# yashsmehta/visreps

Measured on AMD Instinct MI355X. Metric: end-to-end RSA eval sec (extract→RDM→1000-bootstrap Spearman), N=10k stimuli, lower is better.
Workload: dtype bf16x3-split Gram, fp32 accumulate (|dSpearman| < 1e-5 vs fp64 RDMs: tests/test_benchsize.py) / exact int ranks, fp64 statistic

## Files before the change

include/visreps_hip.h:

```cpp
#ifndef VISREPS_HIP_H
#define VISREPS_HIP_H

#include <stddef.h>
#include <stdint.h>

#ifdef __cplusplus
extern "C" {
#endif

#define VR_OK 0
#define VR_EINVAL (-1)
#define VR_EHIP (-2)
#define VR_EWORKSPACE (-3)
#define VR_EINTERNAL (-4)
#define VR_ENOCONV (-5)

int vr_version(void);
const char* vr_last_error(void);

size_t vr_rdm_pearson_workspace(int64_t n, int64_t d);
int vr_rdm_pearson_f32(const float* X, int64_t n, int64_t d, int64_t ldx, float* rdm,
                       int64_t ldr, float correction, void* ws, size_t ws_bytes,
                       void* stream);

// ... 121 lines not shown
                      void* ws, size_t ws_bytes, void* stream);

size_t vr_bootstrap_cka_workspace(int64_t n, int64_t n_sets);
int vr_bootstrap_cka_f32(const float* K, const float* L, int64_t n, int64_t ld,
                         const int32_t* idx, int64_t k, int64_t n_sets, int full_first,
                         double* scores, void* ws, size_t ws_bytes, void* stream);

size_t vr_knn2_workspace(int64_t n, int64_t d);
int vr_knn2_f32(const float* X, int64_t n, int64_t d, int64_t ldx, double* r, int32_t* nn,
                void* ws, size_t ws_bytes, void* stream);
int64_t vr_knn2_last_fallback_rows(void);
int vr_twonn_id_f64(const double* r, int64_t n, double* out, void* stream);

size_t vr_srp_workspace(int64_t B, int64_t D);
int vr_srp_csr_f32(const int32_t* indptr, const int32_t* indices, const float* values,
                   int64_t k, int64_t D, const float* X, int64_t B, int64_t ldx, float* out,
                   int64_t ldo, void* ws, size_t ws_bytes, void* stream);

size_t vr_spearman_full_workspace(int64_t n);
size_t vr_spearman_full_sort_workspace(int64_t n);
int vr_spearman_full_last_form(void);
int vr_spearman_full_f32(const float* A, const float* B, int64_t n, int64_t ld, double* out,
                         void* ws, size_t ws_bytes, void* stream);
int vr_spearman_full_subset_f32(const float* A, const float* B, int64_t n, int64_t ld, const int32_t* idx,
                                int64_t k, double* out, void* ws, size_t ws_bytes, void* stream);
int vr_key_counts_u32(const uint32_t* keys, int64_t m, uint32_t kmin, int64_t bins, uint32_t* cnt, void* stream);
size_t vr_key_table_workspace(int64_t bins);
int vr_key_table_midranks(const uint32_t* keys, int64_t m, uint32_t kmin, uint32_t* cnt, int64_t bins, uint64_t* y,
                          uint64_t* tie, void* ws, size_t ws_bytes, void* stream);
int vr_f32_sort_keys(const float* v, int64_t m, uint32_t* keys, void* stream);
size_t vr_sort_pairs_workspace(int64_t m);
int vr_sort_pairs_u32(uint32_t* keys, uint32_t* vals, int64_t m, void* ws, size_t ws_bytes,
                      void* stream);
size_t vr_midranks_workspace(int64_t m);
int vr_midranks_sorted(const uint32_t* keys, int64_t m, uint64_t base, uint64_t* y, uint64_t* tie,
                       void* ws, size_t ws_bytes, void* stream);
size_t vr_dot_u64_workspace(void);
int vr_dot_u64(const uint64_t* a, const uint64_t* b, int64_t m, uint64_t* out, void* ws,
               size_t ws_bytes, void* stream);

int64_t vr_rdm_plane_rows(int64_t n);
size_t vr_rdm_plane_row_bytes(int64_t d);
int vr_rdm_split_rows_f32(const float* X, int64_t rows, int64_t d, int64_t ldx, float correction,
                          float* mean, float* stdv, uint16_t* planes, void* stream);
int vr_rdm_split_rows_multi_f32(int npts, const float* const* X, const int64_t* d, const int64_t* ldx,
                                int64_t rows, float correction, float* const* mean, float* const* stdv,
                                uint16_t* const* planes, void* stream);
int vr_gather_rows_multi_f32(int npts, const float* const* X, const int64_t* d, const int64_t* ldx,
                             int nrows, const int32_t* src, const int32_t* dst, float* const* out,
                             const int64_t* ldo, void* stream);
size_t vr_rdm_planes_tiles_workspace(int64_t n, int64_t d, int64_t tile_begin, int64_t tile_end);
int vr_rdm_pearson_tiles_planes(const uint16_t* planes, const float* mean, const float* stdv,
                                int64_t n, int64_t d, float* rdm, int64_t ldr, float correction,
                                int64_t tile_begin, int64_t tile_end, void* ws, size_t ws_bytes,
                                void* stream);
int vr_rdm_tiles_pack(const float* rdm, int64_t ldr, int64_t n, int64_t tile_begin,
                      int64_t tile_end, float* packed, void* stream);
int vr_rdm_tiles_unpack(const float* packed, int64_t n, int64_t tile_begin, int64_t tile_end,
                        float* rdm, int64_t ldr, void* stream);

int vr_rccl_available(void);
int vr_rccl_unique_id(void* out );
int vr_rccl_comm_init(void** comm, int world, const void* unique_id, int rank);
int vr_rccl_comm_destroy(void* comm);
int vr_rdm_sharded_range(int64_t n, int64_t d, int world, int rank, int64_t* tile_begin, int64_t* tile_end);
size_t vr_rdm_sharded_workspace(int64_t n, int64_t d, int world);
int vr_rdm_pearson_sharded(const float* X_local, int64_t rows_local, int64_t n, int64_t d, int64_t ldx, float* rdm,
                           int64_t ldr, float correction, void* comm, int rank, int world, void* ws, size_t ws_bytes,
                           void* stream);

typedef int (*vr_allgather_fn)(const void* send, void* recv, size_t bytes, void* user, void* stream);
typedef struct vr_comm {
  int world;
  int rank;
  vr_allgather_fn all_gather;
  void* user;
} vr_comm;
int vr_comm_rccl(vr_comm* out, void* nccl_comm, int world, int rank);
int vr_rdm_pearson_sharded_comm(const float* X_local, int64_t rows_local, int64_t n, int64_t d, int64_t ldx,
                                float* rdm, int64_t ldr, float correction, const vr_comm* comm, void* ws,
                                size_t ws_bytes, void* stream);

size_t vr_transform_workspace(int64_t B, int64_t H, int64_t W, int64_t resize, int64_t crop,
                              int filter);
int vr_transform_u8(const uint8_t* src, int64_t B, int64_t H, int64_t W, int64_t resize,
                    int64_t crop, int filter, const float* mean, const float* std, float* out,
                    void* ws, size_t ws_bytes, void* stream);

int vr_col_sum_f32(const float* X, int64_t n, int64_t p, int64_t ldx, const float* init,
                   float* sum, void* stream);
int vr_col_mean_f32(const float* X, int64_t n, int64_t p, int64_t ldx, float* mean, void* stream);
int vr_mean_from_sum_f32(const float* sum, int64_t p, int64_t n, float* mean, void* stream);
size_t vr_pca_cov_workspace(int64_t n, int64_t p);
int vr_pca_cov_f64(const float* X, int64_t n, int64_t p, int64_t ldx, const float* mean,
                   double denom, double* cov, int64_t ldc, void* ws, size_t ws_bytes,
                   void* stream);

size_t vr_gram64_workspace(int64_t n, int64_t p, int rows);
int vr_gram64_f32(const float* X, int64_t n, int64_t p, int64_t ldx, int rows, double* G, int64_t ldg,
                  void* ws, size_t ws_bytes, void* stream);

int vr_col_mean_f64(const float* X, int64_t n, int64_t p, int64_t ldx, double* mean, void* stream);
size_t vr_centred_gram64_workspace(int64_t n, int64_t p, int rows);
int vr_centred_gram64_f32(const float* X, int64_t n, int64_t p, int64_t ldx, const double* mean,
                          int rows, double denom, double* G, int64_t ldg, void* ws,
                          size_t ws_bytes, void* stream);

size_t vr_eigvalsh_workspace(int64_t m);
int vr_eigvalsh_f64(double* A, int64_t m, int64_t lda, double* w, void* ws, size_t ws_bytes,
                    void* stream);

size_t vr_eigh_top_workspace(int64_t m, int64_t k);
int vr_eigh_top_f64(double* A, int64_t m, int64_t lda, int64_t k, double* w, double* V, int64_t ldv,
                    void* ws, size_t ws_bytes, void* stream);

size_t vr_xgemm_nt_workspace(int64_t M, int64_t N, int64_t K);
int vr_xgemm_nt_f32(const float* A, int64_t M, int64_t K, int64_t lda, const int32_t* a_rows,
                    const double* a_mean, const void* B, int b_f64, int64_t N, int64_t ldb, void* G,
                    int g_f64, int64_t ldg, void* ws, size_t ws_bytes, void* stream);

size_t vr_xcov_segments_workspace(int64_t p, int64_t q, int64_t F, int64_t max_seg);
int vr_xcov_segments_f32(const float* X, int64_t ldx, const float* Y, int64_t ldy, int64_t p, int64_t q,
                         const int32_t* rows, const int64_t* seg, int64_t F, const double* mean_x,
                         const double* mean_y, double* S, double* stats, void* ws, size_t ws_bytes,
                         void* stream);

size_t vr_fold_xcov_workspace(int64_t p, int64_t q);
int vr_fold_xcov_f64(const double* S, const double* stats, const int64_t* seg, int64_t F, int64_t p,
                     int64_t q, const double* mean_x, const double* mean_y, double* C, void* ws,
                     size_t ws_bytes, void* stream);

size_t vr_plssvd_folds_workspace(int64_t p, int64_t q, int64_t k, int64_t max_test);
int vr_plssvd_folds_f64(const float* X, int64_t ldx, const float* Y, int64_t ldy, int64_t p, int64_t q,
                        const int32_t* rows, const int64_t* seg, int64_t F, int64_t n_run,
                        const double* mean_x, const double* mean_y, const double* S, const double* stats,
                        int64_t k, double* corr, double* cov, double* sigma, int32_t* null,
                        double* imbalance, int64_t wfold, double* weights, double* wmean, double* wstd,
                        void* ws, size_t ws_bytes, void* stream);

size_t vr_svd_jacobi_workspace(int64_t batch, int64_t p, int64_t q);
int vr_svd_jacobi_f64(const double* A, int64_t batch, int64_t p, int64_t q, int64_t lda, int64_t stride_a,
                      double* S, double* U, double* Vt, int32_t* null, int32_t* sweeps, void* ws,
                      size_t ws_bytes, void* stream);
int vr_jacobi_schedule(int64_t nb, int32_t* pairs);

size_t vr_plssvd_folds_svd_workspace(int64_t p, int64_t q, int64_t k, int64_t max_test, int64_t n_run);
int vr_plssvd_folds_svd_f64(const float* X, int64_t ldx, const float* Y, int64_t ldy, int64_t p, int64_t q,
                            const int32_t* rows, const int64_t* seg, int64_t F, int64_t n_run,
                            const double* mean_x, const double* mean_y, const double* S, const double* stats,
                            int64_t k, double* corr, double* cov, double* sigma, int32_t* null,
                            double* imbalance, int64_t wfold, double* weights, double* wmean, double* wstd,
                            void* ws, size_t ws_bytes, void* stream);

size_t vr_rng_state_bytes(void);
int vr_rng_seed(void* state, uint32_t seed);
int vr_rng_permutation(void* state, int64_t n, int32_t* out);
int vr_rng_choice(void* state, int64_t n, int64_t k, int32_t* out);
int vr_rng_random_u32(void* state, int64_t count, uint32_t* out);
int vr_rng_normal_f64(void* state, int64_t count, double loc, double scale, double* out);
int vr_legacy_choice(uint32_t seed, int64_t n, int64_t k, int64_t n_draws, int32_t* out);

double vr_percentile_linear(const double* x, int64_t n, double q);

#ifdef __cplusplus
}
#endif

#endif
```

visreps_amd/_lib.py:

```python
from __future__ import annotations

import ctypes
import os
import threading

import torch

__all__ = [
    "LIB_PATH",
    "VisrepsHipError",
    "lib",
    "check",
    "stream_of",
    "workspace",
    "EXPORTED_SYMBOLS",
]

LIB_PATH = os.environ.get("VISREPS_AMD_LIB") or os.path.join(
    os.path.dirname(os.path.abspath(__file__)), "libvisreps_hip.so")


class VisrepsHipError(RuntimeError):
    """A libvisreps_hip call returned a non-zero status."""

# ... 104 lines not shown
        [_vp, _c_i64, _vp, _c_i64, _c_i64, _vp, _c_i64, _c_i64, ctypes.c_int, _vp, _c_i64, _vp, _vp, _c_sz, _vp],
    ),
    "vr_engine_posmap4_bytes": (_c_sz, [_c_i64]),
    "vr_engine_posmap4": (ctypes.c_int, [_vp, _c_i64, _c_i64, _vp, _vp]),
    "vr_engine_join4": (ctypes.c_int, [_vp, _c_i64, _vp, _c_i64, _vp, _vp]),
    "vr_engine_est_reruns": (_c_i64, []),
    "vr_engine_est_tail_flags": (_c_i64, []),
    "vr_test_engine_inject": (ctypes.c_int, [_c_i64]),
    "vr_engine_est_predicted": (_c_i64, []),
    "vr_engine_est1_fallbacks": (_c_i64, []),
    "vr_ktimer_enable": (ctypes.c_int, [ctypes.c_int]),
    "vr_trace_mark": (ctypes.c_int, [ctypes.c_int, ctypes.c_int, _vp]),
    "vr_ktimer_read": (ctypes.c_int, [ctypes.c_int, ctypes.POINTER(ctypes.c_double),
                                      ctypes.POINTER(ctypes.c_int64), ctypes.POINTER(ctypes.c_double)]),
    "vr_bootstrap_spearman_workspace": (_c_sz, [_c_i64]),
    "vr_bootstrap_spearman_f32": (
        ctypes.c_int,
        [_vp, _vp, _c_i64, _c_i64, _vp, _c_i64, _c_i64, ctypes.c_int, _vp, _vp, _c_sz, _vp],
    ),
    "vr_kendall_triu_workspace": (_c_sz, [_c_i64]),
    "vr_kendall_triu_f32": (
        ctypes.c_int,
        [_vp, _vp, _c_i64, _c_i64, _vp, _vp, _c_sz, _vp],
    ),
    "vr_kendall_vec_workspace": (_c_sz, [_c_i64]),
    "vr_kendall_tau_a_f64": (ctypes.c_int, [_vp, _vp, _c_i64, _vp, _vp, _c_sz, _vp]),
    "vr_kendall_full_vec_workspace": (_c_sz, [_c_i64]),
    "vr_kendall_full_vec_f64": (ctypes.c_int, [_vp, _vp, _c_i64, _vp, _vp, _c_sz, _vp]),
    "vr_kendall_full_workspace": (_c_sz, [_c_i64]),
    "vr_kendall_full_f32": (ctypes.c_int, [_vp, _vp, _c_i64, _c_i64, _vp, _vp, _c_sz, _vp]),
    "vr_bootstrap_kendall_workspace": (_c_sz, [_c_i64, _c_i64]),
    "vr_bootstrap_kendall_plans": (
        ctypes.c_int,
        [_vp, _vp, _c_i64, _vp, _c_i64, _c_i64, ctypes.c_int, _vp, _vp, _c_sz, _vp],
    ),
    "vr_srp_workspace": (_c_sz, [_c_i64, _c_i64]),
    "vr_srp_csr_f32": (
        ctypes.c_int,
        [_vp, _vp, _vp, _c_i64, _c_i64, _vp, _c_i64, _c_i64, _vp, _c_i64, _vp, _c_sz, _vp],
    ),
    "vr_col_sum_f32": (ctypes.c_int, [_vp, _c_i64, _c_i64, _c_i64, _vp, _vp, _vp]),
    "vr_col_mean_f32": (ctypes.c_int, [_vp, _c_i64, _c_i64, _c_i64, _vp, _vp]),
    "vr_mean_from_sum_f32": (ctypes.c_int, [_vp, _c_i64, _c_i64, _vp, _vp]),
    "vr_pca_cov_workspace": (_c_sz, [_c_i64, _c_i64]),
    "vr_pca_cov_f64": (
        ctypes.c_int,
        [_vp, _c_i64, _c_i64, _c_i64, _vp, ctypes.c_double, _vp, _c_i64, _vp, _c_sz, _vp],
    ),
    "vr_gram64_workspace": (_c_sz, [_c_i64, _c_i64, ctypes.c_int]),
    "vr_gram64_f32": (ctypes.c_int, [_vp, _c_i64, _c_i64, _c_i64, ctypes.c_int, _vp, _c_i64, _vp, _c_sz, _vp]),
    "vr_col_mean_f64": (ctypes.c_int, [_vp, _c_i64, _c_i64, _c_i64, _vp, _vp]),
    "vr_centred_gram64_workspace": (_c_sz, [_c_i64, _c_i64, ctypes.c_int]),
    "vr_centred_gram64_f32": (
        ctypes.c_int,
        [_vp, _c_i64, _c_i64, _c_i64, _vp, ctypes.c_int, ctypes.c_double, _vp, _c_i64, _vp, _c_sz, _vp],
    ),
    "vr_eigvalsh_workspace": (_c_sz, [_c_i64]),
    "vr_eigvalsh_f64": (ctypes.c_int, [_vp, _c_i64, _c_i64, _vp, _vp, _c_sz, _vp]),
    "vr_eigh_top_workspace": (_c_sz, [_c_i64, _c_i64]),
    "vr_eigh_top_f64": (ctypes.c_int, [_vp, _c_i64, _c_i64, _c_i64, _vp, _vp, _c_i64, _vp, _c_sz, _vp]),
    "vr_spearman_full_workspace": (_c_sz, [_c_i64]),
    "vr_spearman_full_sort_workspace": (_c_sz, [_c_i64]),
    "vr_spearman_full_last_form": (ctypes.c_int, []),
    "vr_key_counts_u32": (ctypes.c_int, [_vp, _c_i64, ctypes.c_uint32, _c_i64, _vp, _vp]),
    "vr_key_table_workspace": (_c_sz, [_c_i64]),
    "vr_key_table_midranks": (ctypes.c_int, [_vp, _c_i64, ctypes.c_uint32, _vp, _c_i64, _vp, _vp, _vp, _c_sz, _vp]),
    "vr_spearman_full_f32": (ctypes.c_int, [_vp, _vp, _c_i64, _c_i64, _vp, _vp, _c_sz, _vp]),
    "vr_spearman_full_subset_f32": (ctypes.c_int, [_vp, _vp, _c_i64, _c_i64, _vp, _c_i64, _vp, _vp, _c_sz, _vp]),
    "vr_kendall_full_subset_f32": (ctypes.c_int, [_vp, _vp, _c_i64, _c_i64, _vp, _c_i64, _vp, _vp, _c_sz, _vp]),
    "vr_f32_sort_keys": (ctypes.c_int, [_vp, _c_i64, _vp, _vp]),
    "vr_sort_pairs_workspace": (_c_sz, [_c_i64]),
    "vr_sort_pairs_u32": (ctypes.c_int, [_vp, _vp, _c_i64, _vp, _c_sz, _vp]),
    "vr_midranks_workspace": (_c_sz, [_c_i64]),
    "vr_midranks_sorted": (ctypes.c_int, [_vp, _c_i64, ctypes.c_uint64, _vp, _vp, _vp, _c_sz, _vp]),
    "vr_dot_u64_workspace": (_c_sz, []),
    "vr_dot_u64": (ctypes.c_int, [_vp, _vp, _c_i64, _vp, _vp, _c_sz, _vp]),
    "vr_rdm_plane_rows": (_c_i64, [_c_i64]),
    "vr_rdm_plane_row_bytes": (_c_sz, [_c_i64]),
    "vr_rdm_split_rows_f32": (
        ctypes.c_int, [_vp, _c_i64, _c_i64, _c_i64, ctypes.c_float, _vp, _vp, _vp, _vp]),
    "vr_rdm_split_rows_multi_f32": (
        ctypes.c_int, [ctypes.c_int, _vp, _vp, _vp, _c_i64, ctypes.c_float, _vp, _vp, _vp, _vp]),
    "vr_gather_rows_multi_f32": (
        ctypes.c_int, [ctypes.c_int, _vp, _vp, _vp, ctypes.c_int, _vp, _vp, _vp, _vp, _vp]),
    "vr_rdm_planes_tiles_workspace": (_c_sz, [_c_i64, _c_i64, _c_i64, _c_i64]),
    "vr_rdm_pearson_tiles_planes": (
        ctypes.c_int,
        [_vp, _vp, _vp, _c_i64, _c_i64, _vp, _c_i64, ctypes.c_float, _c_i64, _c_i64, _vp, _c_sz, _vp],
    ),
    "vr_rccl_available": (ctypes.c_int, []),
    "vr_rccl_unique_id": (ctypes.c_int, [_vp]),
    "vr_rccl_comm_init": (ctypes.c_int, [ctypes.POINTER(ctypes.c_void_p), ctypes.c_int, _vp, ctypes.c_int]),
    "vr_rccl_comm_destroy": (ctypes.c_int, [_vp]),
    "vr_rdm_sharded_range": (ctypes.c_int, [_c_i64, _c_i64, ctypes.c_int, ctypes.c_int,
                                            ctypes.POINTER(ctypes.c_int64), ctypes.POINTER(ctypes.c_int64)]),
    "vr_rdm_sharded_workspace": (_c_sz, [_c_i64, _c_i64, ctypes.c_int]),
    "vr_rdm_pearson_sharded": (
        ctypes.c_int,
        [_vp, _c_i64, _c_i64, _c_i64, _c_i64, _vp, _c_i64, ctypes.c_float, _vp, ctypes.c_int, ctypes.c_int, _vp,
         _c_sz, _vp],
    ),
    "vr_comm_rccl": (ctypes.c_int, [_vp, _vp, ctypes.c_int, ctypes.c_int]),
    "vr_rdm_pearson_sharded_comm": (
        ctypes.c_int,
        [_vp, _c_i64, _c_i64, _c_i64, _c_i64, _vp, _c_i64, ctypes.c_float, _vp, _vp, _c_sz, _vp],
    ),
    "vr_rdm_tiles_pack": (ctypes.c_int, [_vp, _c_i64, _c_i64, _c_i64, _c_i64, _vp, _vp]),
    "vr_rdm_tiles_unpack": (ctypes.c_int, [_vp, _c_i64, _c_i64, _c_i64, _vp, _c_i64, _vp]),
    "vr_transform_workspace": (_c_sz, [_c_i64, _c_i64, _c_i64, _c_i64, _c_i64, ctypes.c_int]),
    "vr_transform_u8": (
        ctypes.c_int,
        [_vp, _c_i64, _c_i64, _c_i64, _c_i64, _c_i64, ctypes.c_int, _vp, _vp, _vp, _vp, _c_sz, _vp],
    ),
    "vr_rng_state_bytes": (_c_sz, []),
    "vr_rng_seed": (ctypes.c_int, [_vp, ctypes.c_uint32]),
    "vr_rng_permutation": (ctypes.c_int, [_vp, _c_i64, _vp]),
    "vr_rng_choice": (ctypes.c_int, [_vp, _c_i64, _c_i64, _vp]),
    "vr_rng_random_u32": (ctypes.c_int, [_vp, _c_i64, _vp]),
    "vr_rng_normal_f64": (ctypes.c_int, [_vp, _c_i64, ctypes.c_double, ctypes.c_double, _vp]),
    "vr_xgemm_nt_workspace": (_c_sz, [_c_i64, _c_i64, _c_i64]),
    "vr_xgemm_nt_f32": (
        ctypes.c_int,
        [_vp, _c_i64, _c_i64, _c_i64, _vp, _vp, _vp, ctypes.c_int, _c_i64, _c_i64, _vp, ctypes.c_int, _c_i64,
         _vp, _c_sz, _vp],
    ),
    "vr_xcov_segments_workspace": (_c_sz, [_c_i64, _c_i64, _c_i64, _c_i64]),
    "vr_xcov_segments_f32": (
        ctypes.c_int,
        [_vp, _c_i64, _vp, _c_i64, _c_i64, _c_i64, _vp, _vp, _c_i64, _vp, _vp, _vp, _vp, _vp, _c_sz, _vp],
    ),
    "vr_fold_xcov_workspace": (_c_sz, [_c_i64, _c_i64]),
    "vr_fold_xcov_f64": (
        ctypes.c_int,
        [_vp, _vp, _vp, _c_i64, _c_i64, _c_i64, _vp, _vp, _vp, _vp, _c_sz, _vp],
    ),
    "vr_plssvd_folds_workspace": (_c_sz, [_c_i64, _c_i64, _c_i64, _c_i64]),
    "vr_plssvd_folds_f64": (
        ctypes.c_int,
        [_vp, _c_i64, _vp, _c_i64, _c_i64, _c_i64, _vp, _vp, _c_i64, _c_i64, _vp, _vp, _vp, _vp, _c_i64,
         _vp, _vp, _vp, _vp, _vp, _c_i64, _vp, _vp, _vp, _vp, _c_sz, _vp],
    ),
    "vr_svd_jacobi_workspace": (_c_sz, [_c_i64, _c_i64, _c_i64]),
    "vr_svd_jacobi_f64": (
        ctypes.c_int,
        [_vp, _c_i64, _c_i64, _c_i64, _c_i64, _c_i64, _vp, _vp, _vp, _vp, _vp, _vp, _c_sz, _vp],
    ),
    "vr_jacobi_schedule": (ctypes.c_int, [_c_i64, _vp]),
    "vr_plssvd_folds_svd_workspace": (_c_sz, [_c_i64, _c_i64, _c_i64, _c_i64, _c_i64]),
    "vr_plssvd_folds_svd_f64": (
        ctypes.c_int,
        [_vp, _c_i64, _vp, _c_i64, _c_i64, _c_i64, _vp, _vp, _c_i64, _c_i64, _vp, _vp, _vp, _vp, _c_i64,
         _vp, _vp, _vp, _vp, _vp, _c_i64, _vp, _vp, _vp, _vp, _c_sz, _vp],
    ),
    "vr_legacy_choice": (ctypes.c_int, [ctypes.c_uint32, _c_i64, _c_i64, _c_i64, _vp]),
    "vr_percentile_linear": (ctypes.c_double, [_vp, _c_i64, ctypes.c_double]),
}

EXPORTED_SYMBOLS = tuple(_PROTOTYPES)

VR_ALLGATHER_FN = ctypes.CFUNCTYPE(ctypes.c_int, _vp, _vp, _c_sz, _vp, _vp)


class VrComm(ctypes.Structure):
    _fields_ = [("world", ctypes.c_int), ("rank", ctypes.c_int), ("all_gather", VR_ALLGATHER_FN), ("user", _vp)]

_lib = None
_lock = threading.Lock()


def lib() -> ctypes.CDLL:
    global _lib
    if _lib is not None:
        return _lib
    with _lock:
        if _lib is None:
            if not os.path.exists(LIB_PATH):
                raise ImportError(
                    f"{LIB_PATH} not found: build the MI355X kernels first "
                    "(python -c 'import __graft_entry__ as g; g.build()' or "
                    "make -C visreps_amd/csrc). There is no CPU fallback."
                )
            handle = ctypes.CDLL(LIB_PATH, mode=ctypes.RTLD_GLOBAL)
            for name, (res, args) in _PROTOTYPES.items():
                fn = getattr(handle, name)
                fn.restype = res
                fn.argtypes = args
            _lib = handle
    return _lib


def check(rc: int, fn: str) -> None:
    if rc != 0:
        msg = lib().vr_last_error().decode(errors="replace")
        raise VisrepsHipError(f"{fn} failed (status {rc}): {msg}")


def stream_of(device: torch.device) -> int:
    return int(torch.cuda.current_stream(device).cuda_stream)


class _WorkspacePool:

    def __init__(self):
        self._bufs: dict[tuple, torch.Tensor] = {}

    def get(self, device: torch.device, nbytes: int, tag: str = "ws") -> torch.Tensor:
        key = (str(device), tag)
        buf = self._bufs.get(key)
        if buf is None or buf.numel() < nbytes:
            self._bufs.pop(key, None)
            buf = torch.empty(max(int(nbytes), 256), dtype=torch.uint8, device=device)
            self._bufs[key] = buf
        return buf

    def current(self, device: torch.device, tag: str = "ws") -> int:
        buf = self._bufs.get((str(device), tag))
        return 0 if buf is None else int(buf.numel())

    def release(self, tag: str | None = None) -> None:
        if tag is None:
            self._bufs.clear()
        else:
            for k in [k for k in self._bufs if k[1] == tag]:
                del self._bufs[k]


workspace = _WorkspacePool()


KTIMER_KERNELS = {"k_rankB_est": 0, "k_rankB_exact": 1, "k_rankA": 2, "k_join": 3,
                  "k_gram_wide": 4, "k_gram_tile": 5, "k_countA": 6, "k_rankB_full": 7,
                  "k_kwalk": 8, "k_cov": 9, "k_join4": 10,
                  "k_full_corr": 11, "k_rankB_grid": 12}
KTIMER_KNN = {"knn_stage": 13, "k_knn_cand": 14, "knn_rerank": 15, "k_knn_exact_rows": 16}

KTIMER_EIG = {"eig_tridiag": 17, "eig_bisect": 18, "eig_invit": 19, "eig_back": 20}

KTIMER_SVD = {"svd_stage": 21, "svd_step": 22, "svd_finish": 23}


def ktimer_enable(on: bool = True) -> None:
    check(lib().vr_ktimer_enable(1 if on else 0), "vr_ktimer_enable")


def ktimer_read(kernel: str) -> tuple[float, int, float]:
    ms, n, u = ctypes.c_double(), ctypes.c_int64(), ctypes.c_double()
    kid = (KTIMER_KERNELS[kernel] if kernel in KTIMER_KERNELS else
           KTIMER_KNN[kernel] if kernel in KTIMER_KNN else
           KTIMER_SVD[kernel] if kernel in KTIMER_SVD else KTIMER_EIG[kernel])
    check(lib().vr_ktimer_read(kid, ctypes.byref(ms), ctypes.byref(n), ctypes.byref(u)),
          "vr_ktimer_read")
    return ms.value, n.value, u.value


def build_id() -> str:
    import hashlib

    with open(LIB_PATH, "rb") as f:
        return hashlib.sha256(f.read()).hexdigest()[:16]
```

visreps_amd/csrc/internal.h:

```cpp
#pragma once

#include "common.h"

namespace vr {

constexpr int SCAN_BS = 256;
constexpr int SCAN_IPT = 16;
constexpr int SCAN_TILE = SCAN_BS * SCAN_IPT;
size_t scan_ws_elems(int64_t n);
int scan_exclusive_u32(const uint32_t* in, uint32_t* out, int64_t n, uint32_t* total_dev,
                       uint32_t* ws, hipStream_t st);

constexpr int RS_BS = 256;
constexpr int RS_IPT = 16;
constexpr int RS_TILE = RS_BS * RS_IPT;
int radix_pass_kv(const uint32_t* ki, const uint32_t* vi, uint32_t* ko, uint32_t* vo, int64_t n,
                  int shift, uint32_t* ws, hipStream_t st);
size_t radix_ws_elems(int64_t n);
int radix_offsets(const uint32_t* ki, int64_t n, int shift, uint32_t* ws, hipStream_t st);
int radix_pass_k(const uint32_t* ki, uint32_t* ko, int64_t n, int shift, uint32_t* ws, hipStream_t st);
int radix_sort_kv(uint32_t* keys, uint32_t* vals, uint32_t* keys_alt, uint32_t* vals_alt,
                  int64_t n, uint32_t* ws, hipStream_t st);

int pearson_two_pass(const float* A, const float* B, int64_t n_or_k, int64_t ld, const int32_t* idx,
                     double* out, double* part, double* mu, hipStream_t st);

int cka_two_pass(const float* K, const float* L, int64_t n_or_k, int64_t ld, const int32_t* idx,
                 double* out, int n_out, double* part, double* mu, hipStream_t st);

int knn_col_mean_f64(const float* X, int64_t n, int64_t d, int64_t ldx, double* mean, hipStream_t st);

template <int BS>
__device__ inline uint32_t block_exclusive_scan(uint32_t v, uint32_t* lds, uint32_t& total) {
  const int lane = threadIdx.x & 63, wid = threadIdx.x >> 6;
  uint32_t x = v;
#pragma unroll
  for (int o = 1; o < 64; o <<= 1) {
    uint32_t y = __shfl_up(x, o, 64);
    if (lane >= o) x += y;
  }
  if (lane == 63) lds[wid] = x;
  __syncthreads();
  if (threadIdx.x == 0) {
    uint32_t s = 0;
    for (int w = 0; w < BS / 64; ++w) {
      uint32_t t = lds[w];
      lds[w] = s;
      s += t;
    }
    lds[BS / 64] = s;
  }
  __syncthreads();
  uint32_t r = x - v + lds[wid];
  total = lds[BS / 64];
  __syncthreads();
  return r;
}

typedef double f64x4 __attribute__((ext_vector_type(4)));
typedef double f64x2 __attribute__((ext_vector_type(2)));
typedef float f32x4 __attribute__((ext_vector_type(4)));

template <int Q>
__device__ inline void block_sum_waves(const double (&v)[Q], double (*red)[4]) {
  const int lane = threadIdx.x & 63, w = threadIdx.x >> 6;
#pragma unroll
  for (int q = 0; q < Q; ++q) {
    double t = v[q];
    for (int o = 32; o > 0; o >>= 1) t += __shfl_down(t, o, 64);
    if (lane == 0) red[q][w] = t;
  }
  __syncthreads();
}

template <bool PAIRS>
__device__ inline double block_sum_total(const double (&r)[4]) {
  return PAIRS ? (r[0] + r[1]) + (r[2] + r[3]) : r[0] + r[1] + r[2] + r[3];
}

template <int Q, bool PAIRS>
__device__ inline void block_sum(const double (&v)[Q], double (*red)[4], double (&out)[Q]) {
  block_sum_waves<Q>(v, red);
#pragma unroll
  for (int q = 0; q < Q; ++q) out[q] = block_sum_total<PAIRS>(red[q]);
}

__device__ inline int64_t xcd_item(int64_t nb) {
  const int64_t b = blockIdx.x, x = b & 7, k = b >> 3, per = nb >> 3, rem = nb & 7;
  return x * per + (x < rem ? x : rem) + k;
}

__device__ inline int lds_pad(int p) { return p + (p >> 5); }

__device__ inline uint32_t f32_sort_key(float f) {
  uint32_t u = __float_as_uint(f);
  if (u == 0x80000000u) u = 0u;
  return (u & 0x80000000u) ? ~u : (u | 0x80000000u);
}

}

namespace vr {
enum KtKernel : int {
  KT_RANKB_EST = 0,
  KT_RANKB_EXACT = 1,
  KT_RANKA = 2,
  KT_JOIN = 3,
  KT_GRAM_WIDE = 4,
  KT_GRAM_TILE = 5,
  KT_COUNTA = 6,
  KT_RANKB_FULL = 7,
  KT_KWALK = 8,
  KT_COV = 9,
  KT_JOIN4 = 10,
  KT_FULL_CORR = 11,
  KT_RANKB_GRID = 12,
  KT_KNN_STAGE = 13,
  KT_KNN_CAND = 14,
  KT_KNN_RERANK = 15,
  KT_KNN_EXACT = 16,
  KT_EIG_TRIDIAG = 17,
  KT_EIG_BISECT = 18,
  KT_EIG_INVIT = 19,
  KT_EIG_BACK = 20,
  KT_SVD_STAGE = 21,
  KT_SVD_STEP = 22,
  KT_SVD_FINISH = 23,
  KT_N = 24
};
bool ktimer_on();
struct KtScope {
  KtScope(int kernel, double units, hipStream_t st);
  ~KtScope();
  int kernel;
  double units;
  hipStream_t st;
  hipEvent_t e0 = nullptr;
};
}
```

visreps_amd/models/custom_model.py:

```python
from __future__ import annotations

import math
from typing import Dict, Optional, Sequence, Tuple

import torch
import torch.nn as nn

_CUSTOM_CONVS: Sequence[Tuple] = (
    (96, 11, 4, 2, (3, 2)),
    (256, 5, 1, 2, (3, 2)),
    (384, 3, 1, 1, None),
    (384, 3, 1, 1, None),
    (256, 3, 1, 1, (3, 2)),
)
_TINY_CONVS: Sequence[Tuple] = (
    (64, 5, 2, 2, (2, 2)),
    (128, 3, 1, 1, None),
    (256, 3, 1, 1, (2, 2)),
    (512, 3, 1, 1, None),
    (512, 3, 1, 1, None),
)


class BaseCNN(nn.Module):

    conv_spec: Sequence[Tuple] = ()
    pool_hw: int = 3
    hidden: int = 4096

    def __init__(self, num_classes=1000, trainable_layers=None, dropout=0.5, pooling_type="max"):
        super().__init__()
        self.num_classes = num_classes
        self.dropout = dropout
        self.pooling_type = pooling_type
        del trainable_layers
        self._build_architecture()
        self._initialize_weights()

    def _pool(self, kernel_size=3, stride=2):
        if self.pooling_type == "max":
            return nn.MaxPool2d(kernel_size=kernel_size, stride=stride)
        return nn.AvgPool2d(kernel_size=kernel_size, stride=stride)

    def _build_architecture(self):
        layers = []
        c_in = 3
        for c_out, k, s, p, pool in self.conv_spec:
            layers += [nn.Conv2d(c_in, c_out, kernel_size=k, stride=s, padding=p, bias=False),
                       nn.BatchNorm2d(c_out), nn.ReLU(inplace=True)]
            if pool is not None:
                layers.append(self._pool(*pool))
            c_in = c_out
        self.features = nn.Sequential(*layers)
        self.adaptive_pool = nn.AdaptiveAvgPool2d((self.pool_hw, self.pool_hw))
        flat = c_in * self.pool_hw * self.pool_hw
        n_cls = self.num_classes if self.num_classes is not None else 1000
        self.classifier = nn.Sequential(
            nn.Dropout(p=self.dropout), nn.Linear(flat, self.hidden), nn.BatchNorm1d(self.hidden),
            nn.ReLU(inplace=True), nn.Dropout(p=self.dropout), nn.Linear(self.hidden, self.hidden),
            nn.BatchNorm1d(self.hidden), nn.ReLU(inplace=True), nn.Linear(self.hidden, n_cls),
        )

    def _initialize_weights(self):
        n_cls = self.num_classes if self.num_classes is not None else 1000
        for m in self.modules():
            if isinstance(m, nn.Conv2d):
                nn.init.kaiming_normal_(m.weight, mode="fan_out", nonlinearity="relu")
            elif isinstance(m, (nn.BatchNorm2d, nn.BatchNorm1d)):
                nn.init.ones_(m.weight)
                nn.init.zeros_(m.bias)
            elif isinstance(m, nn.Linear):
                if m.out_features == n_cls:
                    nn.init.normal_(m.weight, 0, 1.0 / math.sqrt(m.weight.size(1)))
                else:
                    nn.init.kaiming_normal_(m.weight, mode="fan_out", nonlinearity="relu")
                nn.init.zeros_(m.bias)

    def forward(self, x):
        x = self.features(x)
        x = self.adaptive_pool(x)
        return self.classifier(torch.flatten(x, 1))


class CustomCNN(BaseCNN):

    conv_spec = _CUSTOM_CONVS
    pool_hw = 3
    hidden = 4096


class TinyCustomCNN(BaseCNN):

    conv_spec = _TINY_CONVS
    pool_hw = 4
    hidden = 2048

    def __init__(self, num_classes=200, trainable_layers=None, dropout=0.3, pooling_type="max"):
        super().__init__(num_classes, trainable_layers, dropout, pooling_type)
```

Measured before the change: 1.870.

## Add bf16x3-split MFMA implicit-GEMM kernel for 3x3 stride-1 convolutions

Adds a custom HIP implicit-GEMM convolution for 3x3/stride-1/pad-1 layers. The input is repacked into a padded channels-last buffer of bf16 hi/lo records, and the weights are split once and cached. The kernel runs double-buffered LDS tiles with three bf16 MFMA products to approximate fp32 accuracy. The CNN feature extractor now routes eligible convolutions here instead of MIOpen, aiming to cut feature-extraction time, at the cost of an extra repack pass, a per-call workspace allocation and a small precision change.

```diff
diff --git a/include/visreps_hip.h b/include/visreps_hip.h
--- a/include/visreps_hip.h
+++ b/include/visreps_hip.h
@@ -297,6 +297,12 @@
                             double* imbalance, int64_t wfold, double* weights, double* wmean, double* wstd,
                             void* ws, size_t ws_bytes, void* stream);
 
+size_t vr_conv3_weight_bytes(int64_t cout, int64_t cin);
+int vr_conv3_split_weights_f32(const float* weight, int64_t cout, int64_t cin, void* wrec, void* stream);
+size_t vr_conv3_workspace(int64_t batch, int64_t cin, int64_t h, int64_t w);
+int vr_conv3_forward_f32(const float* x, const void* wrec, float* out, int64_t batch, int64_t cin, int64_t h,
+                         int64_t w, int64_t cout, void* ws, size_t ws_bytes, void* stream);
+
 size_t vr_rng_state_bytes(void);
 int vr_rng_seed(void* state, uint32_t seed);
 int vr_rng_permutation(void* state, int64_t n, int32_t* out);
diff --git a/visreps_amd/_lib.py b/visreps_amd/_lib.py
--- a/visreps_amd/_lib.py
+++ b/visreps_amd/_lib.py
@@ -280,6 +280,13 @@
         [_vp, _c_i64, _vp, _c_i64, _c_i64, _c_i64, _vp, _vp, _c_i64, _c_i64, _vp, _vp, _vp, _vp, _c_i64,
          _vp, _vp, _vp, _vp, _vp, _c_i64, _vp, _vp, _vp, _vp, _c_sz, _vp],
     ),
+    "vr_conv3_weight_bytes": (_c_sz, [_c_i64, _c_i64]),
+    "vr_conv3_split_weights_f32": (ctypes.c_int, [_vp, _c_i64, _c_i64, _vp, _vp]),
+    "vr_conv3_workspace": (_c_sz, [_c_i64, _c_i64, _c_i64, _c_i64]),
+    "vr_conv3_forward_f32": (
+        ctypes.c_int,
+        [_vp, _vp, _vp, _c_i64, _c_i64, _c_i64, _c_i64, _c_i64, _vp, _c_sz, _vp],
+    ),
     "vr_legacy_choice": (ctypes.c_int, [ctypes.c_uint32, _c_i64, _c_i64, _c_i64, _vp]),
     "vr_percentile_linear": (ctypes.c_double, [_vp, _c_i64, ctypes.c_double]),
 }
@@ -359,7 +366,8 @@
 KTIMER_KERNELS = {"k_rankB_est": 0, "k_rankB_exact": 1, "k_rankA": 2, "k_join": 3,
                   "k_gram_wide": 4, "k_gram_tile": 5, "k_countA": 6, "k_rankB_full": 7,
                   "k_kwalk": 8, "k_cov": 9, "k_join4": 10,
-                  "k_full_corr": 11, "k_rankB_grid": 12}
+                  "k_full_corr": 11, "k_rankB_grid": 12,
+                  "k_conv3": 24}
 KTIMER_KNN = {"knn_stage": 13, "k_knn_cand": 14, "knn_rerank": 15, "k_knn_exact_rows": 16}
 
 KTIMER_EIG = {"eig_tridiag": 17, "eig_bisect": 18, "eig_invit": 19, "eig_back": 20}
diff --git a/visreps_amd/csrc/conv.hip b/visreps_amd/csrc/conv.hip
--- /dev/null
+++ b/visreps_amd/csrc/conv.hip
@@ -0,0 +1,309 @@
+#include <cstdlib>
+
+#include "internal.h"
+
+namespace vr {
+namespace {
+
+typedef __bf16 bf16x8 __attribute__((ext_vector_type(8)));
+typedef uint32_t u32x4 __attribute__((ext_vector_type(4)));
+typedef float f32x16 __attribute__((ext_vector_type(16)));
+
+constexpr int CK = 32;
+constexpr int CREC = 64;
+constexpr int CROW = 72;
+constexpr int CTM = 128;
+
+__device__ inline u32x4 conv_pack8(const float v[8], bool lo) {
+  uint32_t u[8];
+#pragma unroll
+  for (int j = 0; j < 8; ++j) {
+    const __bf16 hb = (__bf16)v[j];
+    const __bf16 o = lo ? (__bf16)(v[j] - (float)hb) : hb;
+    u[j] = (uint32_t)__builtin_bit_cast(uint16_t, o);
+  }
+  return u32x4{u[0] | (u[1] << 16), u[2] | (u[3] << 16), u[4] | (u[5] << 16), u[6] | (u[7] << 16)};
+}
+
+constexpr int CS_CHUNK = 256;
+constexpr int CS_LD = CS_CHUNK + 1;
+
+}
+
+__global__ __launch_bounds__(256) void k_conv_split_in(const float* __restrict__ x, int C, int H, int W,
+                                                       uint16_t* __restrict__ P) {
+  __shared__ float tile[CK * CS_LD];
+  const int CB = C / CK, Hp = H + 2, Wp = W + 2, HW = H * W;
+  const int64_t img = blockIdx.x / CB;
+  const int cb = (int)(blockIdx.x % CB);
+  const float* src = x + (img * C + (int64_t)cb * CK) * HW;
+  uint16_t* dst = P + (img * Hp * Wp * CB + cb) * CREC;
+  const int64_t rstride = (int64_t)CB * CREC;
+  const int c = threadIdx.x & 7, r0 = threadIdx.x >> 3;
+
+  for (int q = r0; q < Hp * Wp; q += 32) {
+    const int h = q / Wp, w = q - h * Wp;
+    if (h == 0 || h == Hp - 1 || w == 0 || w == Wp - 1)
+      *reinterpret_cast<u32x4*>(dst + q * rstride + c * 8) = u32x4{0u, 0u, 0u, 0u};
+  }
+  const int lane = threadIdx.x & 63, wid = threadIdx.x >> 6;
+  for (int p0 = 0; p0 < HW; p0 += CS_CHUNK) {
+    const int n = min(CS_CHUNK, HW - p0);
+    for (int k = wid; k < CK; k += 4)
+      for (int j = lane; j < n; j += 64) tile[k * CS_LD + j] = src[(int64_t)k * HW + p0 + j];
+    __syncthreads();
+    for (int r = r0; r < n; r += 32) {
+      const int p = p0 + r, h = p / W, w = p - h * W;
+      float v[8];
+#pragma unroll
+      for (int j = 0; j < 8; ++j) v[j] = tile[((c & 3) * 8 + j) * CS_LD + r];
+      *reinterpret_cast<u32x4*>(dst + ((int64_t)(h + 1) * Wp + (w + 1)) * rstride + c * 8) = conv_pack8(v, c >= 4);
+    }
+    __syncthreads();
+  }
+}
+
+__global__ __launch_bounds__(256) void k_conv_split_w(const float* __restrict__ w, int64_t cout, int C,
+                                                      uint16_t* __restrict__ Wr) {
+  const int CB = C / CK;
+  const int64_t idx = (int64_t)blockIdx.x * 256 + threadIdx.x;
+  if (idx >= cout * 9 * CB * 8) return;
+  const int c = (int)(idx & 7);
+  const int64_t rec = idx >> 3;
+  const int cb = (int)(rec % CB), tap = (int)((rec / CB) % 9);
+  const int64_t co = rec / ((int64_t)CB * 9);
+  const int k0 = cb * CK + (c & 3) * 8;
+  float v[8];
+#pragma unroll
+  for (int j = 0; j < 8; ++j) v[j] = w[(co * C + k0 + j) * 9 + tap];
+  *reinterpret_cast<u32x4*>(Wr + rec * CREC + c * 8) = conv_pack8(v, c >= 4);
+}
+
+struct ConvParams {
+  const uint16_t* P;
+  const uint16_t* Wr;
+  float* out;
+  int64_t NP;
+  int H, W, CB, Cout;
+  int ns;
+  int MT;
+};
+
+template <int TN>
+__global__ __launch_bounds__(2 * TN, TN == 128 ? 2 : 1) void k_conv3(ConvParams q) {
+  constexpr int NT = 2 * TN;
+  constexpr int NA = CTM * 8 / NT;
+  constexpr int NB = TN * 8 / NT;
+  constexpr int A_STAGE = CTM * CROW, B_STAGE = TN * CROW;
+  __shared__ __attribute__((aligned(16))) uint16_t lds[2 * (A_STAGE + B_STAGE)];
+  const int id = (int)xcd_remap(blockIdx.x, gridDim.x);
+  const int mt = id % q.MT, nt = id / q.MT;
+  const int m0 = mt * CTM;
+  const int64_t n0 = (int64_t)nt * TN;
+  const int HW = q.H * q.W, Hp = q.H + 2, Wp = q.W + 2;
+
+  const int lane = threadIdx.x & 63, wid = threadIdx.x >> 6;
+  const int wr = wid / (TN / 64), wc = wid % (TN / 64), h = lane >> 5, l32 = lane & 31;
+
+  const uint16_t* pa[NA];
+  const uint16_t* pb[NB];
+#pragma unroll
+  for (int s = 0; s < NA; ++s) {
+    const int f = threadIdx.x + NT * s;
+    const int co = min(m0 + (f >> 3), q.Cout - 1);
+    pa[s] = q.Wr + (int64_t)co * q.ns * CREC + (f & 7) * 8;
+  }
+#pragma unroll
+  for (int s = 0; s < NB; ++s) {
+    const int f = threadIdx.x + NT * s;
+    const int64_t p = min(n0 + (f >> 3), q.NP - 1);
+    const int64_t img = p / HW;
+    const int hw = (int)(p - img * HW), y = hw / q.W, x = hw - y * q.W;
+    pb[s] = q.P + ((img * Hp + y) * Wp + x) * q.CB * CREC + (f & 7) * 8;
+  }
+
+  f32x16 acc[2][2];
+#pragma unroll
+  for (int a = 0; a < 2; ++a)
+#pragma unroll
+    for (int b = 0; b < 2; ++b)
+#pragma unroll
+      for (int e = 0; e < 16; ++e) acc[a][b][e] = 0.f;
+
+  int64_t offa = 0, offb = 0;
+  int in_row = 0;
+  const int row_stages = 3 * q.CB;
+  const int64_t row_skip = (int64_t)(Wp - 3) * q.CB * CREC;
+  u32x4 ga[NA], gb[NB];
+  auto load = [&]() {
+#pragma unroll
+    for (int s = 0; s < NA; ++s) ga[s] = *reinterpret_cast<const u32x4*>(pa[s] + offa);
+#pragma unroll
+    for (int s = 0; s < NB; ++s) gb[s] = *reinterpret_cast<const u32x4*>(pb[s] + offb);
+    offa += CREC;
+    offb += CREC;
+    if (++in_row == row_stages) {
+      in_row = 0;
+      offb += row_skip;
+    }
+  };
+  auto store = [&](uint16_t* buf) {
+#pragma unroll
+    for (int s = 0; s < NA; ++s) {
+      const int f = threadIdx.x + NT * s;
+      *reinterpret_cast<u32x4*>(buf + (f >> 3) * CROW + (f & 7) * 8) = ga[s];
+    }
+#pragma unroll
+    for (int s = 0; s < NB; ++s) {
+      const int f = threadIdx.x + NT * s;
+      *reinterpret_cast<u32x4*>(buf + A_STAGE + (f >> 3) * CROW + (f & 7) * 8) = gb[s];
+    }
+  };
+
+  load();
+  store(lds);
+  __syncthreads();
+  for (int kt = 0; kt < q.ns; ++kt) {
+    const int cur = kt & 1;
+    const uint16_t* As = lds + cur * (A_STAGE + B_STAGE);
+    const uint16_t* Bs = As + A_STAGE;
+    const bool more = kt + 1 < q.ns;
+    if (more) load();
+#pragma unroll
+    for (int t = 0; t < 2; ++t) {
+      bf16x8 aH[2], aL[2], bH[2], bL[2];
+#pragma unroll
+      for (int m = 0; m < 2; ++m) {
+        const uint16_t* ar = As + (wr * 64 + m * 32 + l32) * CROW + t * 16 + h * 8;
+        const uint16_t* br = Bs + (wc * 64 + m * 32 + l32) * CROW + t * 16 + h * 8;
+        aH[m] = __builtin_bit_cast(bf16x8, *reinterpret_cast<const u32x4*>(ar));
+        aL[m] = __builtin_bit_cast(bf16x8, *reinterpret_cast<const u32x4*>(ar + 32));
+        bH[m] = __builtin_bit_cast(bf16x8, *reinterpret_cast<const u32x4*>(br));
+        bL[m] = __builtin_bit_cast(bf16x8, *reinterpret_cast<const u32x4*>(br + 32));
+      }
+#pragma unroll
+      for (int m = 0; m < 2; ++m)
+#pragma unroll
+        for (int nn = 0; nn < 2; ++nn)
+          acc[m][nn] = __builtin_amdgcn_mfma_f32_32x32x16_bf16(aH[m], bH[nn], acc[m][nn], 0, 0, 0);
+#pragma unroll
+      for (int m = 0; m < 2; ++m)
+#pragma unroll
+        for (int nn = 0; nn < 2; ++nn)
+          acc[m][nn] = __builtin_amdgcn_mfma_f32_32x32x16_bf16(aH[m], bL[nn], acc[m][nn], 0, 0, 0);
+#pragma unroll
+      for (int m = 0; m < 2; ++m)
+#pragma unroll
+        for (int nn = 0; nn < 2; ++nn)
+          acc[m][nn] = __builtin_amdgcn_mfma_f32_32x32x16_bf16(aL[m], bH[nn], acc[m][nn], 0, 0, 0);
+    }
+    if (more) store(lds + (cur ^ 1) * (A_STAGE + B_STAGE));
+    __syncthreads();
+  }
+
+#pragma unroll
+  for (int nn = 0; nn < 2; ++nn) {
+    const int64_t p = n0 + wc * 64 + nn * 32 + l32;
+    if (p >= q.NP) continue;
+    const int64_t img = p / HW;
+    float* o = q.out + img * q.Cout * HW + (p - img * HW);
+#pragma unroll
+    for (int m = 0; m < 2; ++m)
+#pragma unroll
+      for (int r = 0; r < 16; ++r) {
+        const int co = m0 + wr * 64 + m * 32 + (r & 3) + 8 * (r >> 2) + 4 * h;
+        if (co < q.Cout) o[(int64_t)co * HW] = acc[m][nn][r];
+      }
+  }
+}
+
+static size_t conv_image_bytes(int64_t batch, int64_t cin, int64_t h, int64_t w) {
+  return (size_t)batch * (size_t)(h + 2) * (size_t)(w + 2) * (size_t)(cin / CK) * CREC * sizeof(uint16_t);
+}
+
+static int conv_tile(int64_t np, int64_t cout) {
+  static const int forced = [] {
+    const char* e = getenv("VISREPS_CONV_TILE");
+    const int v = e ? atoi(e) : 0;
+    return (v == 128 || v == 256) ? v : 0;
+  }();
+  if (forced) return forced;
+  const int64_t mt = (cout + CTM - 1) / CTM;
+  return mt * ((np + 255) / 256) >= (int64_t)num_cus() * 7 / 8 ? 256 : 128;
+}
+
+}
+
+using namespace vr;
+
+extern "C" {
+
+size_t vr_conv3_weight_bytes(int64_t cout, int64_t cin) {
+  if (cout <= 0 || cin <= 0 || cin % CK) return 0;
+  return (size_t)cout * 9 * (size_t)(cin / CK) * CREC * sizeof(uint16_t);
+}
+
+int vr_conv3_split_weights_f32(const float* weight, int64_t cout, int64_t cin, void* wrec, void* stream) {
+  VR_REQUIRE(cout > 0 && cin > 0 && cin % CK == 0, "vr_conv3_split_weights_f32: cout=%lld, cin=%lld (a multiple of 32)",
+             (long long)cout, (long long)cin);
+  VR_REQUIRE(weight && wrec, "vr_conv3_split_weights_f32: null pointer");
+  VR_REQUIRE(cin <= 0x7fffffff && cout * 9 * (cin / CK) * 8 / 256 < 0x7fffffff, "vr_conv3_split_weights_f32: too large");
+  const int64_t n = cout * 9 * (cin / CK) * 8;
+  k_conv_split_w<<<(unsigned)((n + 255) / 256), 256, 0, as_stream(stream)>>>(weight, cout, (int)cin,
+                                                                               static_cast<uint16_t*>(wrec));
+  VR_CHECK_LAUNCH();
+  return VR_OK;
+}
+
+size_t vr_conv3_workspace(int64_t batch, int64_t cin, int64_t h, int64_t w) {
+  if (batch <= 0 || cin <= 0 || cin % CK || h <= 0 || w <= 0) return 0;
+  return (conv_image_bytes(batch, cin, h, w) + 255) / 256 * 256;
+}
+
+int vr_conv3_forward_f32(const float* x, const void* wrec, float* out, int64_t batch, int64_t cin, int64_t h,
+                         int64_t w, int64_t cout, void* ws, size_t ws_bytes, void* stream) {
+  VR_REQUIRE(batch >= 0 && cin > 0 && cin % CK == 0 && h > 0 && w > 0 && cout > 0,
+             "vr_conv3_forward_f32: batch=%lld cin=%lld (a multiple of 32) h=%lld w=%lld cout=%lld",
+             (long long)batch, (long long)cin, (long long)h, (long long)w, (long long)cout);
+  if (batch == 0) return VR_OK;
+  VR_REQUIRE(x && wrec && out, "vr_conv3_forward_f32: null pointer");
+  const int64_t cb = cin / CK, np = batch * h * w;
+  VR_REQUIRE(h <= 32768 && w <= 32768 && h * w <= (1 << 24) && cin <= (1 << 20) && cout <= (1 << 20) &&
+                 batch * cb < 0x7fffffff && np < ((int64_t)1 << 36),
+             "vr_conv3_forward_f32: shape too large");
+  const size_t need = vr_conv3_workspace(batch, cin, h, w);
+  if (ws == nullptr || ws_bytes < need) {
+    set_error("vr_conv3_forward_f32: workspace %zu < %zu", ws_bytes, need);
+    return VR_EWORKSPACE;
+  }
+  hipStream_t st = as_stream(stream);
+  uint16_t* P = static_cast<uint16_t*>(ws);
+  k_conv_split_in<<<(unsigned)(batch * cb), 256, 0, st>>>(x, (int)cin, (int)h, (int)w, P);
+  VR_CHECK_LAUNCH();
+
+  ConvParams q;
+  q.P = P;
+  q.Wr = static_cast<const uint16_t*>(wrec);
+  q.out = out;
+  q.NP = np;
+  q.H = (int)h;
+  q.W = (int)w;
+  q.CB = (int)cb;
+  q.Cout = (int)cout;
+  q.ns = (int)(9 * cb);
+  q.MT = (int)((cout + CTM - 1) / CTM);
+  const int tn = conv_tile(np, cout);
+  const int64_t nb = (int64_t)q.MT * ((np + tn - 1) / tn);
+  VR_REQUIRE(nb < 0x7fffffff, "vr_conv3_forward_f32: grid too large");
+  {
+    KtScope kt(KT_CONV3, 2.0 * (double)cout * (double)np * (double)cin * 9.0, st);
+    if (tn == 256)
+      k_conv3<256><<<(unsigned)nb, 512, 0, st>>>(q);
+    else
+      k_conv3<128><<<(unsigned)nb, 256, 0, st>>>(q);
+  }
+  VR_CHECK_LAUNCH();
+  return VR_OK;
+}
+
+}
diff --git a/visreps_amd/csrc/internal.h b/visreps_amd/csrc/internal.h
--- a/visreps_amd/csrc/internal.h
+++ b/visreps_amd/csrc/internal.h
@@ -126,7 +126,8 @@
   KT_SVD_STAGE = 21,
   KT_SVD_STEP = 22,
   KT_SVD_FINISH = 23,
-  KT_N = 24
+  KT_CONV3 = 24,
+  KT_N = 25
 };
 bool ktimer_on();
 struct KtScope {
diff --git a/visreps_amd/models/custom_model.py b/visreps_amd/models/custom_model.py
--- a/visreps_amd/models/custom_model.py
+++ b/visreps_amd/models/custom_model.py
@@ -1,6 +1,8 @@
 from __future__ import annotations
 
+import ctypes
 import math
+import os
 from typing import Dict, Optional, Sequence, Tuple
 
 import torch
@@ -20,6 +22,67 @@
     (512, 3, 1, 1, None),
     (512, 3, 1, 1, None),
 )
+
+
+SPLIT_MIN_TILES = 64
+
+
+def split_conv_tiles(c_out: int, batch: int, h: int, w: int) -> int:
+    return -(-c_out // 128) * -(-(batch * h * w) // 128)
+
+
+class SplitConv2d(nn.Conv2d):
+
+    def _native_ok(self, x: torch.Tensor) -> bool:
+        w = self.weight
+        return (x.is_cuda and x.dim() == 4 and x.dtype == torch.float32 and w.dtype == torch.float32
+                and w.device == x.device and x.is_contiguous() and w.is_contiguous()
+                and self.bias is None and self.kernel_size == (3, 3) and self.stride == (1, 1)
+                and self.padding == (1, 1) and self.dilation == (1, 1) and self.groups == 1
+                and self.padding_mode == "zeros" and self.in_channels % 32 == 0
+                and x.shape[1] == self.in_channels and x.numel() > 0
+                and not (torch.is_grad_enabled() and (x.requires_grad or w.requires_grad))
+                and self._mode_ok(x))
+
+    def _mode_ok(self, x: torch.Tensor) -> bool:
+        mode = os.environ.get("VISREPS_CONV", "")
+        if mode == "miopen":
+            return False
+        return mode == "split" or split_conv_tiles(self.out_channels, x.shape[0], x.shape[2], x.shape[3]) >= SPLIT_MIN_TILES
+
+    def _weight_records(self, L, stream) -> torch.Tensor:
+        w = self.weight
+        key = (w.untyped_storage().data_ptr(), w.storage_offset(), w.device, w._version)
+        cached = self.__dict__.get("_wrec")
+        if cached is not None and cached[0] == key:
+            return cached[1]
+        from .._lib import check
+
+        co, ci = self.out_channels, self.in_channels
+        rec = torch.empty(int(L.vr_conv3_weight_bytes(co, ci)), dtype=torch.uint8, device=w.device)
+        check(L.vr_conv3_split_weights_f32(ctypes.c_void_p(w.data_ptr()), co, ci, ctypes.c_void_p(rec.data_ptr()),
+                                           ctypes.c_void_p(stream)), "vr_conv3_split_weights_f32")
+        self.__dict__["_wrec"] = (key, rec)
+        return rec
+
+    def forward(self, x: torch.Tensor) -> torch.Tensor:
+        if not self._native_ok(x):
+            return super().forward(x)
+        from .._lib import check, lib, stream_of
+
+        L = lib()
+        b, ci, h, w = x.shape
+        with torch.cuda.device(x.device):
+            stream = stream_of(x.device)
+            rec = self._weight_records(L, stream)
+            ws_bytes = int(L.vr_conv3_workspace(b, ci, h, w))
+            ws = torch.empty(ws_bytes, dtype=torch.uint8, device=x.device)
+            out = torch.empty((b, self.out_channels, h, w), dtype=torch.float32, device=x.device)
+            check(L.vr_conv3_forward_f32(ctypes.c_void_p(x.data_ptr()), ctypes.c_void_p(rec.data_ptr()),
+                                         ctypes.c_void_p(out.data_ptr()), b, ci, h, w, self.out_channels,
+                                         ctypes.c_void_p(ws.data_ptr()), ws_bytes, ctypes.c_void_p(stream)),
+                  "vr_conv3_forward_f32")
+        return out
 
 
 class BaseCNN(nn.Module):
@@ -46,7 +109,7 @@
         layers = []
         c_in = 3
         for c_out, k, s, p, pool in self.conv_spec:
-            layers += [nn.Conv2d(c_in, c_out, kernel_size=k, stride=s, padding=p, bias=False),
+            layers += [SplitConv2d(c_in, c_out, kernel_size=k, stride=s, padding=p, bias=False),
                        nn.BatchNorm2d(c_out), nn.ReLU(inplace=True)]
             if pool is not None:
                 layers.append(self._pool(*pool))
```

After: 2.015. 1.08x slower.
